# myshell-ai/OpenVoice

Hardware: NVIDIA H100
Metric: audio_seconds_per_second (higher is better)
Workload: dtype f32 (3xFP16 split-precision tensor-core convs with fp32 accumulation, fp32 FFMA elsewhere)

## Files before the change

openvoice_b200/csrc/ovc_tcconv.cuh:

```cuda
#pragma once
#include "ovc_conv.cuh"
#include "ovc_tc.cuh"
#include "ovc_tcpack.h"

namespace ovc {

struct TcConvArgs {
  const float* x; long long x_bs;
  const uint16_t* w;
  const float* bias; long long bias_bs;
  float* y; long long y_bs; int y_ld;
  const float* r;
  float* s; long long s_bs;
  int epi;
  int split; int first;
  const long long* lens; int tmax; int mul;
  const long long* lens_x; int has_lens_x;
  int Cin; int Ntot; int K; int DIL;
  float slope; float scale; int accumulate;
  int passes;
  const uint16_t* w2; const float* bias2;
};

__device__ __forceinline__ void pdl_launch_dependents() { asm volatile("griddepcontrol.launch_dependents;" ::: "memory"); }
__device__ __forceinline__ void pdl_wait() { asm volatile("griddepcontrol.wait;" ::: "memory"); }

__device__ __forceinline__ void mbar_arrive(uint64_t* bar) {
  asm volatile("mbarrier.arrive.shared::cta.b64 _, [%0];" ::"r"(smem_u32(bar)) : "memory");
}
__device__ __forceinline__ void named_bar_sync(int id, int threads) {
  asm volatile("bar.sync %0, %1;" ::"r"(id), "r"(threads) : "memory");
}

template <int TN>
__device__ __forceinline__ void tc_epilogue(const TcConvArgs& a, const float (&d)[TN], int b, int t0, int n0, int lim, int row_a) {
  const int csub = (threadIdx.x & 3) * 2;
  float* yb = a.y + (size_t)b * a.y_bs;
  const float* rb = a.r ? a.r + (size_t)b * a.y_bs : nullptr;
  float* sb = a.s ? a.s + (size_t)b * a.s_bs : nullptr;
  const float* bias = a.bias + (size_t)b * a.bias_bs;
  const bool two = a.passes == 3;
  const int ta = t0 + row_a, tb = ta + 8;
  const bool oka = ta < lim, okb = tb < lim;
#pragma unroll
  for (int c0 = 0; c0 < TN; c0 += 32) {
    float v[16];
#pragma unroll
    for (int i = 0; i < 16; ++i) v[i] = two ? fmaf(d[TN / 2 + c0 / 2 + i], tc::kLoInv, d[c0 / 2 + i]) : d[c0 / 2 + i];
#pragma unroll
    for (int g = 0; g < 4; ++g) {
      const float2 bq = __ldg(reinterpret_cast<const float2*>(bias + n0 + c0 + 8 * g + csub));
      v[4 * g] += bq.x; v[4 * g + 1] += bq.y; v[4 * g + 2] += bq.x; v[4 * g + 3] += bq.y;
    }
    if (a.epi == 0) {
      float* ypa = yb + (size_t)ta * a.y_ld + n0 + c0 + csub;
      float* ypb = yb + (size_t)tb * a.y_ld + n0 + c0 + csub;
      const float* rpa = rb ? rb + (size_t)ta * a.y_ld + n0 + c0 + csub : nullptr;
      const float* rpb = rb ? rb + (size_t)tb * a.y_ld + n0 + c0 + csub : nullptr;
#pragma unroll
      for (int g = 0; g < 4; ++g) {
        float2 oa = make_float2(v[4 * g], v[4 * g + 1]), ob = make_float2(v[4 * g + 2], v[4 * g + 3]);
        if (rb) {
          const float2 qa = oka ? *reinterpret_cast<const float2*>(rpa + 8 * g) : make_float2(0.f, 0.f);
          const float2 qb = okb ? *reinterpret_cast<const float2*>(rpb + 8 * g) : make_float2(0.f, 0.f);
          oa.x += qa.x; oa.y += qa.y; ob.x += qb.x; ob.y += qb.y;
        }
        if (a.accumulate) {
          const float2 ya = oka ? *reinterpret_cast<const float2*>(ypa + 8 * g) : make_float2(0.f, 0.f);
          const float2 yc = okb ? *reinterpret_cast<const float2*>(ypb + 8 * g) : make_float2(0.f, 0.f);
          oa.x = ya.x + oa.x; oa.y = ya.y + oa.y;
          ob.x = yc.x + ob.x; ob.y = yc.y + ob.y;
        }
        if (a.scale != 1.f) { oa.x *= a.scale; oa.y *= a.scale; ob.x *= a.scale; ob.y *= a.scale; }
        if (oka) *reinterpret_cast<float2*>(ypa + 8 * g) = oa;
        if (okb) *reinterpret_cast<float2*>(ypb + 8 * g) = ob;
      }
    } else if (a.epi == 1) {
      float* ypa = yb + (size_t)ta * a.y_ld + ((n0 + c0) >> 1) + csub;
      float* ypb = yb + (size_t)tb * a.y_ld + ((n0 + c0) >> 1) + csub;
#pragma unroll
      for (int g = 0; g < 2; ++g) {
        const float2 oa = make_float2(tanhf(v[4 * g]) * sigmoidf_acc(v[4 * (g + 2)]),
                                      tanhf(v[4 * g + 1]) * sigmoidf_acc(v[4 * (g + 2) + 1]));
        const float2 ob = make_float2(tanhf(v[4 * g + 2]) * sigmoidf_acc(v[4 * (g + 2) + 2]),
                                      tanhf(v[4 * g + 3]) * sigmoidf_acc(v[4 * (g + 2) + 3]));
        if (oka) *reinterpret_cast<float2*>(ypa + 8 * g) = oa;
        if (okb) *reinterpret_cast<float2*>(ypb + 8 * g) = ob;
      }
    } else {
      const int col = n0 + c0;
      const bool to_x = col < a.split;
      const bool add = to_x || !a.first;
      float* dst = (to_x ? yb + col : sb + (col - a.split)) + csub;
#pragma unroll
      for (int g = 0; g < 4; ++g) {
        float2 oa = make_float2(v[4 * g], v[4 * g + 1]), ob = make_float2(v[4 * g + 2], v[4 * g + 3]);
        if (add) {
          const float2 qa = oka ? *reinterpret_cast<const float2*>(dst + (size_t)ta * a.y_ld + 8 * g) : make_float2(0.f, 0.f);
          const float2 qb = okb ? *reinterpret_cast<const float2*>(dst + (size_t)tb * a.y_ld + 8 * g) : make_float2(0.f, 0.f);
          oa = make_float2(qa.x + oa.x, qa.y + oa.y);
          ob = make_float2(qb.x + ob.x, qb.y + ob.y);
        }
        if (oka) *reinterpret_cast<float2*>(dst + (size_t)ta * a.y_ld + 8 * g) = oa;
        if (okb) *reinterpret_cast<float2*>(dst + (size_t)tb * a.y_ld + 8 * g) = ob;
      }
    }
  }
}

template <int TN>
__device__ __forceinline__ void tc_mma_step(float (&d)[TN], uint64_t a_hi, uint64_t a_lo, uint64_t b, bool three, bool first) {
  float (&lo)[TN / 2] = *reinterpret_cast<float(*)[TN / 2]>(&d[TN / 2]);
  float (&hi)[TN / 2] = *reinterpret_cast<float(*)[TN / 2]>(&d[0]);
  tc::Wgmma<TN>::mma(hi, a_hi, b, first ? 0 : 1);
  if (three) {
    tc::Wgmma<TN>::mma(lo, a_hi, b + TN, first ? 0 : 1);
    tc::Wgmma<TN>::mma(lo, a_lo, b, 1);
  }
}

constexpr int TCN_THREADS = 384;
constexpr int TCN_NCT = 96;

template <int TN, bool PAIR>
struct TcnCfg {
  static_assert(!PAIR || TN == 32 || TN == 64, "conv pairs: C = 32 or 64");
  static constexpr int KCH = 32, NKC = KCH / 8;
  static constexpr int ROWS = 194;
  static constexpr int ROWS2 = 146;
  static constexpr int NABUF = 2;
  static constexpr int RING = tc_ring_slots(TN, PAIR);
  static constexpr int SLOT_BYTES = 2 * 2 * TN * 16;
  static constexpr int A_BUF_BYTES = 2 * NKC * ROWS * 16;
  static constexpr int A2_BYTES = PAIR ? 2 * (TN / 8) * ROWS2 * 16 : 0;
  static constexpr size_t SMEM_BYTES = 1024 + NABUF * A_BUF_BYTES + A2_BYTES + RING * SLOT_BYTES;
  static_assert(SMEM_BYTES <= 232448, "shared memory budget");
  static_assert((2 * NABUF + 2 * RING) * 8 <= 1024, "barrier area");
};

constexpr int TCN_PROD_REGS = 56, TCN_MMA_REGS = 224;

template <int TN, bool PAIR>
__global__ void __launch_bounds__(TCN_THREADS, 1) tcconv_kernel(const TcConvArgs a, int n_tt, int total) {
  using Cfg = TcnCfg<TN, PAIR>;
  constexpr int ROWS = Cfg::ROWS, ROWS2 = Cfg::ROWS2, NABUF = Cfg::NABUF, RING = Cfg::RING, NKC = Cfg::NKC;
  extern __shared__ __align__(128) unsigned char smem_raw[];
  uint64_t* bars = reinterpret_cast<uint64_t*>(smem_raw);
  uint64_t *a_full = bars, *a_empty = bars + NABUF, *b_full = a_empty + NABUF, *b_empty = b_full + RING;
  unsigned char* abuf = smem_raw + 1024;
  unsigned char* a2buf = abuf + NABUF * Cfg::A_BUF_BYTES;
  unsigned char* bring = a2buf + Cfg::A2_BYTES;

  const int tid = threadIdx.x, lane = tid & 31;
  const int warp = __shfl_sync(0xffffffffu, tid >> 5, 0);
  const int H1 = (a.K - 1) / 2 * a.DIL;
  const int H2 = PAIR ? (a.K - 1) / 2 : 0;
  const int R = 128 - 2 * H2;
  const int rows8 = (128 + 2 * H1 + 7) & ~7;
  const int nq = a.Cin / Cfg::KCH;
  const int n_slots = (a.Cin / 16) * a.K;
  const int n_w = PAIR ? 2 * n_slots : n_slots;
  const bool resident = n_w <= RING;
  if (H1 > TCN_HMAX || (PAIR && (!resident || 128 + 2 * H2 > ROWS2))) __trap();
  constexpr uint32_t BYTES = Cfg::SLOT_BYTES;

  if (tid == 0) {
    for (int i = 0; i < NABUF; ++i) { mbar_init(&a_full[i], TCN_NCT); mbar_init(&a_empty[i], 2); }
    for (int i = 0; i < RING; ++i) { mbar_init(&b_full[i], 1); mbar_init(&b_empty[i], 2); }
    fence_mbar_init();
  }
  if (PAIR) {
    for (int i = tid; i < Cfg::A2_BYTES / 16; i += TCN_THREADS) reinterpret_cast<uint4*>(a2buf)[i] = make_uint4(0u, 0u, 0u, 0u);
    asm volatile("fence.proxy.async.shared::cta;" ::: "memory");
  }
  __syncthreads();
  pdl_launch_dependents();
  if (warp != 0) pdl_wait();

#define TCN_FOR_TILES                                                                                   \
  for (int tile = blockIdx.x; tile < total; tile += gridDim.x) {                                        \
    const int b = tile / n_tt, t0 = (tile % n_tt) * R;                                                  \
    const int lim = (a.lens ? (int)min((long long)a.tmax, a.lens[b]) : a.tmax) * a.mul;                 \
    const int lim_x = a.has_lens_x ? (int)min((long long)a.tmax, a.lens_x[b]) * a.mul : lim;            \
    (void)lim_x;                                                                                        \
    if (t0 >= lim) continue;

  if (warp < 4) {
    tc::regs_dealloc<TCN_PROD_REGS>();
    if (warp == 0) {
      if (lane == 0) {
        const unsigned char* wt = reinterpret_cast<const unsigned char*>(a.w) + (size_t)blockIdx.y * n_slots * BYTES;
        if (resident) {
          for (int it = 0; it < n_w; ++it) {
            const unsigned char* src = it < n_slots ? wt + (size_t)it * BYTES
                                                    : reinterpret_cast<const unsigned char*>(a.w2) + (size_t)(it - n_slots) * BYTES;
            mbar_expect_tx(&b_full[it], BYTES);
            tma_bulk_g2s(bring + it * BYTES, src, BYTES, &b_full[it]);
          }
          for (int it = 0; it < n_w; ++it) mbar_wait(&b_full[it], 0u);
        } else {
          int slot = 0;
          uint32_t phase = 1;
          TCN_FOR_TILES
            (void)b;
            for (int it = 0; it < n_slots; ++it) {
              mbar_wait(&b_empty[slot], phase);
              mbar_expect_tx(&b_full[slot], BYTES);
              tma_bulk_g2s(bring + slot * BYTES, wt + (size_t)it * BYTES, BYTES, &b_full[slot]);
              if (++slot == RING) { slot = 0; phase ^= 1; }
            }
          }
        }
      }
    } else {
      const int pt = tid - 32;
      const int items = rows8 * NKC;
      int buf = 0;
      uint32_t ephase = 1;
      TCN_FOR_TILES
        const float* xb = a.x + (size_t)b * a.x_bs;
        const int r0 = t0 - H2 - H1;
        for (int q = 0; q < nq; ++q) {
          mbar_wait(&a_empty[buf], ephase);
          unsigned char* ah = abuf + buf * Cfg::A_BUF_BYTES;
          unsigned char* al = ah + NKC * ROWS * 16;
          constexpr int PB = 2;
          for (int i0 = pt; i0 < items; i0 += TCN_NCT * PB) {
            float4 v0[PB], v1[PB];
#pragma unroll
            for (int u = 0; u < PB; ++u) {
              const int i = i0 + TCN_NCT * u;
              const int row = i >> 2, kc = i & 3;
              const int t = r0 + row;
              v0[u] = make_float4(0.f, 0.f, 0.f, 0.f);
              v1[u] = v0[u];
              if (i < items && t >= 0 && t < lim_x) {
                const float4* src = reinterpret_cast<const float4*>(xb + (size_t)t * a.Cin + q * Cfg::KCH + kc * 8);
                v0[u] = src[0];
                v1[u] = src[1];
              }
            }
#pragma unroll
            for (int u = 0; u < PB; ++u) {
              const int i = i0 + TCN_NCT * u;
              if (i >= items) break;
              const int row = i >> 2, kc = i & 3;
              uint4 hi, lo;
              tc::split_f16x8(v0[u], v1[u], a.slope, hi, lo);
              *reinterpret_cast<uint4*>(ah + (kc * ROWS + row) * 16) = hi;
              *reinterpret_cast<uint4*>(al + (kc * ROWS + row) * 16) = lo;
            }
          }
          asm volatile("fence.proxy.async.shared::cta;" ::: "memory");
          mbar_arrive(&a_full[buf]);
          if (++buf == NABUF) { buf = 0; ephase ^= 1; }
        }
      }
    }
  } else {
    tc::regs_alloc<TCN_MMA_REGS>();
    const int wg = (warp >> 2) - 1;
    const bool leader = (tid & 127) == 0;
    const int row_a = 64 * wg + 16 * (warp & 3) + (lane >> 2);
    constexpr uint32_t LBO_A = ROWS * 16, LBO_A2 = ROWS2 * 16, LBO_B = 2 * TN * 16, SBO = 128;
    constexpr uint32_t A_LO16 = (NKC * ROWS * 16) >> 4, A2_LO16 = ((TN / 8) * ROWS2 * 16) >> 4, SLOT16 = BYTES >> 4;
    const uint64_t a_proto = tc::make_desc(0, LBO_A, SBO), b_proto = tc::make_desc(0, LBO_B, SBO);
    const uint64_t b_ring = b_proto + (tc::smem_addr(bring) >> 4);
    const bool three = a.passes == 3;
    float d[TN];
#pragma unroll
    for (int i = 0; i < TN; ++i) d[i] = 0.f;
    if (resident)
      for (int it = 0; it < n_w; ++it) mbar_wait(&b_full[it], 0u);
    int slot = 0, buf = 0;
    uint32_t bphase = 0, aphase = 0;
    TCN_FOR_TILES
      (void)lim_x;
      bool first = true;
      if (resident) slot = 0;
      for (int q = 0; q < nq; ++q) {
        mbar_wait(&a_full[buf], aphase);
        tc::fence_regs(d);
        tc::wgmma_fence();
        int prev = -1;
        for (int j = 0; j < 2; ++j) {
          uint64_t a_cur = a_proto + ((tc::smem_addr(abuf + buf * Cfg::A_BUF_BYTES) + 64 * wg * 16 + 2 * j * LBO_A) >> 4);
          for (int tap = 0; tap < a.K; ++tap) {
            if (!resident) mbar_wait(&b_full[slot], bphase);
            tc_mma_step<TN>(d, a_cur, a_cur + A_LO16, b_ring + (uint32_t)slot * SLOT16, three, first);
            tc::wgmma_commit();
            if (!resident) {
              tc::wgmma_wait<1>();
              if (leader && prev >= 0) mbar_arrive(&b_empty[prev]);
              prev = slot;
            }
            first = false;
            a_cur += a.DIL;
            if (++slot == RING) { slot = 0; bphase ^= 1; }
          }
        }
        tc::wgmma_wait<0>();
        tc::fence_regs(d);
        if (leader) {
          if (prev >= 0) mbar_arrive(&b_empty[prev]);
          mbar_arrive(&a_empty[buf]);
        }
        if (++buf == NABUF) { buf = 0; aphase ^= 1; }
      }
      if constexpr (!PAIR) {
        tc_epilogue<TN>(a, d, b, t0, blockIdx.y * TN, lim, row_a);
      } else {
        named_bar_sync(1, 256);
        unsigned char* a2h = a2buf;
        unsigned char* a2l = a2buf + (TN / 8) * ROWS2 * 16;
        const int ta = t0 - H2 + row_a, tb = ta + 8;
        const bool oka = ta >= 0 && ta < lim, okb = tb >= 0 && tb < lim;
        const int csub = (lane & 3) * 2;
#pragma unroll
        for (int g = 0; g < TN / 8; ++g) {
          const float2 bq = __ldg(reinterpret_cast<const float2*>(a.bias + 8 * g + csub));
          float x[4];
#pragma unroll
          for (int i = 0; i < 4; ++i) x[i] = (three ? fmaf(d[TN / 2 + 4 * g + i], tc::kLoInv, d[4 * g + i]) : d[4 * g + i]) + ((i & 1) ? bq.y : bq.x);
          x[0] = oka ? fmaxf(x[0], x[0] * a.slope) : 0.f;
          x[1] = oka ? fmaxf(x[1], x[1] * a.slope) : 0.f;
          x[2] = okb ? fmaxf(x[2], x[2] * a.slope) : 0.f;
          x[3] = okb ? fmaxf(x[3], x[3] * a.slope) : 0.f;
          const __half2 ha = __floats2half2_rn(x[0], x[1]), hb = __floats2half2_rn(x[2], x[3]);
          const float2 fa = __half22float2(ha), fb = __half22float2(hb);
          const __half2 la = __floats2half2_rn((x[0] - fa.x) * tc::kLoScale, (x[1] - fa.y) * tc::kLoScale);
          const __half2 lb = __floats2half2_rn((x[2] - fb.x) * tc::kLoScale, (x[3] - fb.y) * tc::kLoScale);
          const int oa = (g * ROWS2 + row_a) * 16 + (lane & 3) * 4, ob = oa + 8 * 16;
          *reinterpret_cast<__half2*>(a2h + oa) = ha;
          *reinterpret_cast<__half2*>(a2h + ob) = hb;
          *reinterpret_cast<__half2*>(a2l + oa) = la;
          *reinterpret_cast<__half2*>(a2l + ob) = lb;
        }
        asm volatile("fence.proxy.async.shared::cta;" ::: "memory");
        named_bar_sync(2, 256);
        const uint64_t a2_proto = tc::make_desc(0, LBO_A2, SBO);
        tc::fence_regs(d);
        tc::wgmma_fence();
        bool first2 = true;
        for (int kk = 0; kk < TN / 16; ++kk) {
          uint64_t a_cur = a2_proto + ((tc::smem_addr(a2buf) + 64 * wg * 16 + 2 * kk * LBO_A2) >> 4);
          for (int tap = 0; tap < a.K; ++tap) {
            tc_mma_step<TN>(d, a_cur, a_cur + A2_LO16, b_ring + (uint32_t)(n_slots + kk * a.K + tap) * SLOT16, three, first2);
            first2 = false;
            a_cur += 1;
          }
        }
        tc::wgmma_commit();
        tc::wgmma_wait<0>();
        tc::fence_regs(d);
        TcConvArgs e = a;
        e.y_ld = TN; e.r = a.x; e.bias = a.bias2; e.bias_bs = 0; e.epi = 0;
        tc_epilogue<TN>(e, d, b, t0, 0, min(lim, t0 + R), row_a);
      }
    }
  }
#undef TCN_FOR_TILES
}

template <int C>
__global__ void __launch_bounds__(256) conv_post_cl_kernel(const float* __restrict__ x, long long x_bs,
                                                           const float* __restrict__ w, float* __restrict__ y,
                                                           long long y_bs, int y_len, const long long* lens, int tmax,
                                                           int mul) {
  constexpr int TB = 256, ROWS = TB + 6, LD = ROWS + 3;
  __shared__ float ws[7][C];
  __shared__ float xs[C][LD];
  for (int i = threadIdx.x; i < C * 7; i += blockDim.x) ws[i % 7][i / 7] = w[i];
  const int b = blockIdx.y;
  const int lim = (lens ? (int)min((long long)tmax, lens[b]) : tmax) * mul;
  const int t0 = blockIdx.x * TB;
  const float* xb = x + (size_t)b * x_bs;
  for (int idx = threadIdx.x; idx < ROWS * (C / 4); idx += blockDim.x) {
    const int row = idx / (C / 4), q = idx % (C / 4);
    const int tt = t0 - 3 + row;
    float4 v = make_float4(0.f, 0.f, 0.f, 0.f);
    if (tt >= 0 && tt < lim) v = *reinterpret_cast<const float4*>(xb + (size_t)tt * C + 4 * q);
    xs[4 * q + 0][row] = v.x > 0.f ? v.x : 0.01f * v.x;
    xs[4 * q + 1][row] = v.y > 0.f ? v.y : 0.01f * v.y;
    xs[4 * q + 2][row] = v.z > 0.f ? v.z : 0.01f * v.z;
    xs[4 * q + 3][row] = v.w > 0.f ? v.w : 0.01f * v.w;
  }
  __syncthreads();
  const int t = t0 + threadIdx.x;
  if (t >= y_len) return;
  float acc = 0.f;
  if (t < lim) {
#pragma unroll
    for (int k = 0; k < 7; ++k)
#pragma unroll 8
      for (int ci = 0; ci < C; ++ci) acc = fmaf(ws[k][ci], xs[ci][threadIdx.x + k], acc);
    acc = tanhf(acc);
  }
  y[(size_t)b * y_bs + t] = acc;
}

__global__ void __launch_bounds__(256) transpose_kernel(const float* __restrict__ src, float* __restrict__ dst, int rows,
                                                        int cols, long long bs) {
  __shared__ float tile[32][33];
  const float* s = src + (size_t)blockIdx.z * bs;
  float* d = dst + (size_t)blockIdx.z * bs;
  const int c0 = blockIdx.x * 32, r0 = blockIdx.y * 32;
  const int tx = threadIdx.x & 31, ty = threadIdx.x >> 5;
  for (int i = ty; i < 32; i += 8) {
    const int r = r0 + i, c = c0 + tx;
    tile[i][tx] = (r < rows && c < cols) ? s[(size_t)r * cols + c] : 0.f;
  }
  __syncthreads();
  for (int i = ty; i < 32; i += 8) {
    const int c = c0 + i, r = r0 + tx;
    if (r < rows && c < cols) d[(size_t)c * rows + r] = tile[tx][i];
  }
}

}
```

Before: 1983.

## Stage activations with cp.async ring and prefetch epilogue residuals before MMA

The producer warps now stage raw fp32 input chunks into a multi-slot shared-memory ring with cp.async, running several chunks (and tiles) ahead. They then convert from shared memory into the split fp16 A buffers, which hides global-load latency behind conversion. For TN<=64 the MMA warpgroups load the residual and accumulate operands into registers before the MMA loop, so those loads no longer stall the epilogue. This costs extra shared memory and register pressure, and the A-buffer row count is now derived from TCN_HMAX.

```diff
diff --git a/openvoice_b200/csrc/ovc_tcconv.cuh b/openvoice_b200/csrc/ovc_tcconv.cuh
--- a/openvoice_b200/csrc/ovc_tcconv.cuh
+++ b/openvoice_b200/csrc/ovc_tcconv.cuh
@@ -32,11 +32,49 @@
   asm volatile("bar.sync %0, %1;" ::"r"(id), "r"(threads) : "memory");
 }
 
+struct TcEpiIn {
+  float2 p[8], q[8];
+};
+__device__ __forceinline__ void tc_epi_fetch(const TcConvArgs& a, TcEpiIn& in, int b, int t0, int col, int lim, int row_a) {
+  const int csub = (threadIdx.x & 3) * 2;
+  const int ta = t0 + row_a, tb = ta + 8;
+  const bool oka = ta < lim, okb = tb < lim;
+  const float* pp = nullptr;
+  const float* qp = nullptr;
+  if (a.epi == 0) {
+    if (a.r) pp = a.r + (size_t)b * a.y_bs + col;
+    if (a.accumulate) qp = a.y + (size_t)b * a.y_bs + col;
+  } else if (a.epi == 2) {
+    const bool to_x = col < a.split;
+    if (to_x || !a.first) pp = to_x ? a.y + (size_t)b * a.y_bs + col : a.s + (size_t)b * a.s_bs + (col - a.split);
+  }
+#pragma unroll
+  for (int g = 0; g < 4; ++g) {
+    const size_t oa = (size_t)ta * a.y_ld + 8 * g + csub, ob = (size_t)tb * a.y_ld + 8 * g + csub;
+    in.p[2 * g] = pp && oka ? *reinterpret_cast<const float2*>(pp + oa) : make_float2(0.f, 0.f);
+    in.p[2 * g + 1] = pp && okb ? *reinterpret_cast<const float2*>(pp + ob) : make_float2(0.f, 0.f);
+    in.q[2 * g] = qp && oka ? *reinterpret_cast<const float2*>(qp + oa) : make_float2(0.f, 0.f);
+    in.q[2 * g + 1] = qp && okb ? *reinterpret_cast<const float2*>(qp + ob) : make_float2(0.f, 0.f);
+  }
+}
+
 template <int TN>
-__device__ __forceinline__ void tc_epilogue(const TcConvArgs& a, const float (&d)[TN], int b, int t0, int n0, int lim, int row_a) {
+struct TcEpiPre {
+  static constexpr bool EARLY = TN <= 64;
+  TcEpiIn g[EARLY ? TN / 32 : 1];
+  __device__ __forceinline__ void fetch(const TcConvArgs& a, int b, int t0, int n0, int lim, int row_a) {
+    if constexpr (EARLY) {
+#pragma unroll
+      for (int c0 = 0; c0 < TN; c0 += 32) tc_epi_fetch(a, g[c0 / 32], b, t0, n0 + c0, lim, row_a);
+    }
+  }
+};
+
+template <int TN>
+__device__ __forceinline__ void tc_epilogue(const TcConvArgs& a, const float (&d)[TN], const TcEpiPre<TN>& pre, int b, int t0,
+                                            int n0, int lim, int row_a) {
   const int csub = (threadIdx.x & 3) * 2;
   float* yb = a.y + (size_t)b * a.y_bs;
-  const float* rb = a.r ? a.r + (size_t)b * a.y_bs : nullptr;
   float* sb = a.s ? a.s + (size_t)b * a.s_bs : nullptr;
   const float* bias = a.bias + (size_t)b * a.bias_bs;
   const bool two = a.passes == 3;
@@ -44,6 +82,9 @@
   const bool oka = ta < lim, okb = tb < lim;
 #pragma unroll
   for (int c0 = 0; c0 < TN; c0 += 32) {
+    TcEpiIn late;
+    if constexpr (!TcEpiPre<TN>::EARLY) tc_epi_fetch(a, late, b, t0, n0 + c0, lim, row_a);
+    const TcEpiIn& in = TcEpiPre<TN>::EARLY ? pre.g[c0 / 32] : late;
     float v[16];
 #pragma unroll
     for (int i = 0; i < 16; ++i) v[i] = two ? fmaf(d[TN / 2 + c0 / 2 + i], tc::kLoInv, d[c0 / 2 + i]) : d[c0 / 2 + i];
@@ -55,19 +96,15 @@
     if (a.epi == 0) {
       float* ypa = yb + (size_t)ta * a.y_ld + n0 + c0 + csub;
       float* ypb = yb + (size_t)tb * a.y_ld + n0 + c0 + csub;
-      const float* rpa = rb ? rb + (size_t)ta * a.y_ld + n0 + c0 + csub : nullptr;
-      const float* rpb = rb ? rb + (size_t)tb * a.y_ld + n0 + c0 + csub : nullptr;
 #pragma unroll
       for (int g = 0; g < 4; ++g) {
         float2 oa = make_float2(v[4 * g], v[4 * g + 1]), ob = make_float2(v[4 * g + 2], v[4 * g + 3]);
-        if (rb) {
-          const float2 qa = oka ? *reinterpret_cast<const float2*>(rpa + 8 * g) : make_float2(0.f, 0.f);
-          const float2 qb = okb ? *reinterpret_cast<const float2*>(rpb + 8 * g) : make_float2(0.f, 0.f);
+        if (a.r) {
+          const float2 qa = in.p[2 * g], qb = in.p[2 * g + 1];
           oa.x += qa.x; oa.y += qa.y; ob.x += qb.x; ob.y += qb.y;
         }
         if (a.accumulate) {
-          const float2 ya = oka ? *reinterpret_cast<const float2*>(ypa + 8 * g) : make_float2(0.f, 0.f);
-          const float2 yc = okb ? *reinterpret_cast<const float2*>(ypb + 8 * g) : make_float2(0.f, 0.f);
+          const float2 ya = in.q[2 * g], yc = in.q[2 * g + 1];
           oa.x = ya.x + oa.x; oa.y = ya.y + oa.y;
           ob.x = yc.x + ob.x; ob.y = yc.y + ob.y;
         }
@@ -96,8 +133,7 @@
       for (int g = 0; g < 4; ++g) {
         float2 oa = make_float2(v[4 * g], v[4 * g + 1]), ob = make_float2(v[4 * g + 2], v[4 * g + 3]);
         if (add) {
-          const float2 qa = oka ? *reinterpret_cast<const float2*>(dst + (size_t)ta * a.y_ld + 8 * g) : make_float2(0.f, 0.f);
-          const float2 qb = okb ? *reinterpret_cast<const float2*>(dst + (size_t)tb * a.y_ld + 8 * g) : make_float2(0.f, 0.f);
+          const float2 qa = in.p[2 * g], qb = in.p[2 * g + 1];
           oa = make_float2(qa.x + oa.x, qa.y + oa.y);
           ob = make_float2(qb.x + ob.x, qb.y + ob.y);
         }
@@ -121,22 +157,44 @@
 
 constexpr int TCN_THREADS = 384;
 constexpr int TCN_NCT = 96;
+constexpr int TCN_SMEM_MAX = 232448;
 
 template <int TN, bool PAIR>
 struct TcnCfg {
   static_assert(!PAIR || TN == 32 || TN == 64, "conv pairs: C = 32 or 64");
   static constexpr int KCH = 32, NKC = KCH / 8;
-  static constexpr int ROWS = 194;
+  static constexpr int RAW_ROWS = (128 + 2 * TCN_HMAX + 7) & ~7;
+  static constexpr int ROWS = RAW_ROWS + 2;
   static constexpr int ROWS2 = 146;
   static constexpr int NABUF = 2;
   static constexpr int RING = tc_ring_slots(TN, PAIR);
   static constexpr int SLOT_BYTES = 2 * 2 * TN * 16;
   static constexpr int A_BUF_BYTES = 2 * NKC * ROWS * 16;
   static constexpr int A2_BYTES = PAIR ? 2 * (TN / 8) * ROWS2 * 16 : 0;
-  static constexpr size_t SMEM_BYTES = 1024 + NABUF * A_BUF_BYTES + A2_BYTES + RING * SLOT_BYTES;
-  static_assert(SMEM_BYTES <= 232448, "shared memory budget");
+  static constexpr int RAW_BYTES = RAW_ROWS * KCH * 4;
+  static constexpr size_t BASE_BYTES = 1024 + NABUF * A_BUF_BYTES + A2_BYTES + RING * SLOT_BYTES;
+  static constexpr int NRAW = (TCN_SMEM_MAX - BASE_BYTES) / RAW_BYTES >= 3 ? 3 : 2;
+  static constexpr size_t SMEM_BYTES = BASE_BYTES + NRAW * RAW_BYTES;
+  static_assert(ROWS % 8 == 2, "A pitch = 2 (mod 8): conflict-free converter stores");
+  static_assert(SMEM_BYTES <= TCN_SMEM_MAX, "shared memory budget");
   static_assert((2 * NABUF + 2 * RING) * 8 <= 1024, "barrier area");
 };
+
+struct TcTile {
+  int b, t0, lim, lim_x;
+};
+__device__ __forceinline__ TcTile tc_tile(const TcConvArgs& a, int tile, int n_tt, int R) {
+  TcTile s;
+  s.b = tile / n_tt;
+  s.t0 = (tile % n_tt) * R;
+  s.lim = (a.lens ? (int)min((long long)a.tmax, a.lens[s.b]) : a.tmax) * a.mul;
+  s.lim_x = a.has_lens_x ? (int)min((long long)a.tmax, a.lens_x[s.b]) * a.mul : s.lim;
+  return s;
+}
+
+__device__ __forceinline__ void cp_async_commit() { asm volatile("cp.async.commit_group;" ::: "memory"); }
+template <int N>
+__device__ __forceinline__ void cp_async_wait() { asm volatile("cp.async.wait_group %0;" ::"n"(N) : "memory"); }
 
 constexpr int TCN_PROD_REGS = 56, TCN_MMA_REGS = 224;
 
@@ -179,10 +237,8 @@
 
 #define TCN_FOR_TILES                                                                                   \
   for (int tile = blockIdx.x; tile < total; tile += gridDim.x) {                                        \
-    const int b = tile / n_tt, t0 = (tile % n_tt) * R;                                                  \
-    const int lim = (a.lens ? (int)min((long long)a.tmax, a.lens[b]) : a.tmax) * a.mul;                 \
-    const int lim_x = a.has_lens_x ? (int)min((long long)a.tmax, a.lens_x[b]) * a.mul : lim;            \
-    (void)lim_x;                                                                                        \
+    const TcTile tl_ = tc_tile(a, tile, n_tt, R);                                                       \
+    const int b = tl_.b, t0 = tl_.t0, lim = tl_.lim;                                                    \
     if (t0 >= lim) continue;
 
   if (warp < 4) {
@@ -213,47 +269,64 @@
         }
       }
     } else {
+      constexpr int NRAW = Cfg::NRAW;
       const int pt = tid - 32;
       const int items = rows8 * NKC;
-      int buf = 0;
+      unsigned char* raw = bring + RING * BYTES;
+      int st = blockIdx.x, sq = 0, sst = 0;
+      TcTile sl{};
+      auto seek = [&]() {
+        for (; st < total; st += gridDim.x) {
+          sl = tc_tile(a, st, n_tt, R);
+          if (sl.t0 < sl.lim) break;
+        }
+      };
+      seek();
+      auto stage_next = [&]() {
+        if (st < total) {
+          const float* xc = a.x + (size_t)sl.b * a.x_bs + sq * Cfg::KCH;
+          const int r0 = sl.t0 - H2 - H1;
+          unsigned char* dst = raw + sst * Cfg::RAW_BYTES;
+          for (int i = pt; i < items; i += TCN_NCT) {
+            const int t = r0 + (i >> 2);
+            const bool ok = t >= 0 && t < sl.lim_x;
+            const float* src = ok ? xc + (size_t)t * a.Cin + (i & 3) * 8 : a.x;
+            cp_async16_zfill(dst + i * 32, src, ok ? 16u : 0u);
+            cp_async16_zfill(dst + i * 32 + 16, ok ? src + 4 : src, ok ? 16u : 0u);
+          }
+          if (++sq == nq) {
+            sq = 0;
+            st += gridDim.x;
+            seek();
+          }
+        }
+        cp_async_commit();
+        if (++sst == NRAW) sst = 0;
+      };
+      for (int s = 0; s < NRAW - 1; ++s) stage_next();
+      int buf = 0, cst = 0;
       uint32_t ephase = 1;
       TCN_FOR_TILES
-        const float* xb = a.x + (size_t)b * a.x_bs;
-        const int r0 = t0 - H2 - H1;
+        (void)b; (void)t0;
         for (int q = 0; q < nq; ++q) {
+          stage_next();
+          cp_async_wait<NRAW - 1>();
           mbar_wait(&a_empty[buf], ephase);
           unsigned char* ah = abuf + buf * Cfg::A_BUF_BYTES;
           unsigned char* al = ah + NKC * ROWS * 16;
-          constexpr int PB = 2;
-          for (int i0 = pt; i0 < items; i0 += TCN_NCT * PB) {
-            float4 v0[PB], v1[PB];
-#pragma unroll
-            for (int u = 0; u < PB; ++u) {
-              const int i = i0 + TCN_NCT * u;
-              const int row = i >> 2, kc = i & 3;
-              const int t = r0 + row;
-              v0[u] = make_float4(0.f, 0.f, 0.f, 0.f);
-              v1[u] = v0[u];
-              if (i < items && t >= 0 && t < lim_x) {
-                const float4* src = reinterpret_cast<const float4*>(xb + (size_t)t * a.Cin + q * Cfg::KCH + kc * 8);
-                v0[u] = src[0];
-                v1[u] = src[1];
-              }
-            }
-#pragma unroll
-            for (int u = 0; u < PB; ++u) {
-              const int i = i0 + TCN_NCT * u;
-              if (i >= items) break;
-              const int row = i >> 2, kc = i & 3;
-              uint4 hi, lo;
-              tc::split_f16x8(v0[u], v1[u], a.slope, hi, lo);
-              *reinterpret_cast<uint4*>(ah + (kc * ROWS + row) * 16) = hi;
-              *reinterpret_cast<uint4*>(al + (kc * ROWS + row) * 16) = lo;
-            }
+          const unsigned char* src = raw + cst * Cfg::RAW_BYTES;
+          for (int i = pt; i < items; i += TCN_NCT) {
+            const int row = i >> 2, kc = i & 3;
+            uint4 hi, lo;
+            tc::split_f16x8(*reinterpret_cast<const float4*>(src + i * 32), *reinterpret_cast<const float4*>(src + i * 32 + 16),
+                            a.slope, hi, lo);
+            *reinterpret_cast<uint4*>(ah + (kc * ROWS + row) * 16) = hi;
+            *reinterpret_cast<uint4*>(al + (kc * ROWS + row) * 16) = lo;
           }
           asm volatile("fence.proxy.async.shared::cta;" ::: "memory");
           mbar_arrive(&a_full[buf]);
           if (++buf == NABUF) { buf = 0; ephase ^= 1; }
+          if (++cst == NRAW) cst = 0;
         }
       }
     }
@@ -272,10 +345,15 @@
     for (int i = 0; i < TN; ++i) d[i] = 0.f;
     if (resident)
       for (int it = 0; it < n_w; ++it) mbar_wait(&b_full[it], 0u);
+    TcConvArgs e = a;
+    if constexpr (PAIR) { e.y_ld = TN; e.r = a.x; e.bias = a.bias2; e.bias_bs = 0; e.epi = 0; }
+    const int n0 = PAIR ? 0 : blockIdx.y * TN;
     int slot = 0, buf = 0;
     uint32_t bphase = 0, aphase = 0;
     TCN_FOR_TILES
-      (void)lim_x;
+      const int elim = PAIR ? min(lim, t0 + R) : lim;
+      TcEpiPre<TN> pre;
+      pre.fetch(e, b, t0, n0, elim, row_a);
       bool first = true;
       if (resident) slot = 0;
       for (int q = 0; q < nq; ++q) {
@@ -308,7 +386,7 @@
         if (++buf == NABUF) { buf = 0; aphase ^= 1; }
       }
       if constexpr (!PAIR) {
-        tc_epilogue<TN>(a, d, b, t0, blockIdx.y * TN, lim, row_a);
+        tc_epilogue<TN>(e, d, pre, b, t0, n0, elim, row_a);
       } else {
         named_bar_sync(1, 256);
         unsigned char* a2h = a2buf;
@@ -353,9 +431,7 @@
         tc::wgmma_commit();
         tc::wgmma_wait<0>();
         tc::fence_regs(d);
-        TcConvArgs e = a;
-        e.y_ld = TN; e.r = a.x; e.bias = a.bias2; e.bias_bs = 0; e.epi = 0;
-        tc_epilogue<TN>(e, d, b, t0, 0, min(lim, t0 + R), row_a);
+        tc_epilogue<TN>(e, d, pre, b, t0, n0, elim, row_a);
       }
     }
   }
```

Measured after the change: 2137 (median of 6 runs). +7.8%, better.
